# infergo-ml/gogp

Hardware: AMD Instinct MI355X
Metric: GP.Observe+Gradient evals/sec (fp64) at N=16384 D=8 (higher is better)
Workload: dtype f64

## Files before the change

gogp_amd/_lib.py:

```python
from __future__ import annotations

import ctypes
import os
import subprocess

from .kernel import CDesc

_HERE = os.path.dirname(os.path.abspath(__file__))
LIB_PATH = os.path.join(_HERE, "libgogp_hip.so")
HOOKS_PATH = os.path.join(_HERE, "libgogp_testhooks.so")

GOGP_OK, GOGP_EARG, GOGP_ENOTPD, GOGP_EHIP, GOGP_ESTATE, GOGP_ENOMEM, GOGP_ECOND = 0, 1, 2, 3, 4, 5, 6
GOGP_MAX_CANDIDATES = 16
GOGP_BATCH_MAX_N = 128
GOGP_COV_MAX_M = 4096
GOGP_MULTI_MAX_T = 128
GOGP_SPARSE_MAX_M = 4096

_dp = ctypes.POINTER(ctypes.c_double)
_i64 = ctypes.c_int64
_h = ctypes.c_void_p
_descp = ctypes.POINTER(CDesc)
GOGP_UNIQUE_ID_BYTES = 128


class CXfer(ctypes.Structure):
    _fields_ = [("peer", ctypes.c_int32), ("is_send", ctypes.c_int32), ("buf", ctypes.c_void_p),
                ("bytes", ctypes.c_int64)]


EXCHANGE_FN = ctypes.CFUNCTYPE(ctypes.c_int, ctypes.c_void_p, ctypes.POINTER(CXfer), ctypes.c_int32)
ALLREDUCE_FN = ctypes.CFUNCTYPE(ctypes.c_int, ctypes.c_void_p, ctypes.POINTER(ctypes.c_double),
                                ctypes.c_int64)
class CGemmOpts(ctypes.Structure):
    _fields_ = [(n, ctypes.c_int32) for n in ("ktri", "krag0", "new_row0", "kbeg0", "small_below", "prio", "rule",
                                              "tpb_shift", "rblk0", "cblk0", "pr", "Pr", "pc", "Pc", "beta0", "k")]
    _fields_ += [("bstride", ctypes.c_int64)]
    DEFAULTS = dict(ktri=0, krag0=-1, new_row0=-1, kbeg0=0, small_below=384, prio=0, rule=0, tpb_shift=0, rblk0=0,
                    cblk0=0, pr=0, Pr=1, pc=0, Pc=1, beta0=-1, k=1, bstride=0)


class CKParams(ctypes.Structure):
    _T, _D, _E = 4, 64, 32
    _fields_ = [("ndim", ctypes.c_int32), ("nterms", ctypes.c_int32), ("kind", ctypes.c_int32 * _T),
                ("ard", ctypes.c_int32 * _T), ("c", ctypes.c_double * _T), ("w", ctypes.c_double * _T),
                ("inv_len", (ctypes.c_double * _D) * _T), ("noise_var", ctypes.c_double), ("dnoise", ctypes.c_double),
                ("nevents", ctypes.c_int32), ("ev_axis", ctypes.c_int32), ("ev_from", ctypes.c_double * _E),
                ("ev_to", ctypes.c_double * _E), ("ev_disc", ctypes.c_double * _E)]


GOGP_TEST_NACC = 16 + 64


class CGemmPlan(ctypes.Structure):
    _fields_ = [("tile", ctypes.c_int32), ("waves", ctypes.c_int32), ("grid_x", ctypes.c_int64),
                ("grid_z", ctypes.c_int64), ("flops", ctypes.c_double), ("tag", ctypes.c_int64)]


SYMBOLS = [
    ("gogp_desc_check", ctypes.c_int, [_descp]),
    ("gogp_desc_ntheta_noise", ctypes.c_int, [_descp]),
    ("gogp_create", ctypes.c_int, [_descp, ctypes.c_int, ctypes.POINTER(_h)]),
    ("gogp_destroy", None, [_h]),
    ("gogp_last_error", ctypes.c_char_p, [_h]),
    ("gogp_notpd_index", _i64, [_h]),
    ("gogp_graph_info", ctypes.c_int, [_h, ctypes.POINTER(ctypes.c_int64), ctypes.POINTER(ctypes.c_int)]),
    ("gogp_events_check", ctypes.c_int, [_dp, ctypes.c_int, ctypes.c_int, ctypes.c_int]),
    ("gogp_set_events", ctypes.c_int, [_h, _dp, ctypes.c_int, ctypes.c_int]),
    ("gogp_set_data", ctypes.c_int, [_h, _dp, _dp, _i64]),
    ("gogp_set_data_device", ctypes.c_int, [_h, ctypes.c_void_p, ctypes.c_void_p, _i64]),
    ("gogp_absorb", ctypes.c_int, [_h, _dp, _dp]),
    ("gogp_observe", ctypes.c_int, [_h, _dp, _i64, _dp]),
# ... 200 lines not shown
```

gogp_amd/csrc/api.hip:

```cpp
#include <math.h>
#include <stdio.h>
#include <stdlib.h>
#include <string.h>

#include <algorithm>
#include <initializer_list>
#include <mutex>
#include <new>
#include <thread>
#include <type_traits>
#include <utility>

#include "handle.h"

using namespace gogp;

static thread_local std::string g_create_error;

extern "C" int gogp_desc_ntheta_noise(const gogp_desc *d) {
  return (d && (d->noise_kind == GOGP_NOISE_UNIFORM || d->noise_kind == GOGP_NOISE_CONSTANT_PARAM)) ? 1 : 0;
}

extern "C" int gogp_desc_check(const gogp_desc *d) {
  if (!d) return GOGP_EARG;
// ... 616 lines not shown
        ldc1[b] = PANEL;
        K1[b] = d * PANEL;
        A2[b] = Dinv + (size_t)i * PANEL * PANEL;
        lda2[b] = PANEL;
        B2[b] = C1[b];
        ldb2[b] = PANEL;
        C2[b] = X + (int64_t)i * PANEL * tld + (int64_t)j * PANEL;
        ldc2[b] = tld;
        K2[b] = PANEL;
      }
      launch_blockmm(sp, nb, A1, lda1, B1, ldb1, C1, ldc1, K1, 1.0);
      launch_blockmm(sp, nb, A2, lda2, B2, ldb2, C2, ldc2, K2, -1.0);
    }
  }
}

template <class T>
struct InvBufs {
  T *A, *Y;
  const T *L, *Dinv;
};
template <class T>
static void trtri_superstep(gogp_handle *h, const InvBufs<T> &B, const SuperPanel &P, hipStream_t st, hipStream_t s2) {
  const int64_t npad = h->npad, ld = npad;
  T *R = B.A, *Y = B.Y;
  const T *L = B.L;
  GemmProfile *pf = &h->prof;
  const int P0 = P.P0;
  const int64_t C0 = P.C0(), CE = P.CE();
  for (int q = 0; q < P.nsub; ++q) {
    const int p = P0 + q;
    const int64_t c0 = (int64_t)p * PANEL, c2 = c0 + PANEL;
    const T *Dp = B.Dinv + (size_t)p * PANEL * PANEL;
    launch_ydiag(st, Dp, Y + c0 * ld + c0, ld);
    if (c2 < CE)
      launch_zero_block(st, Y + c2 * ld + c0, ld, CE - c2, PANEL);
    if (c0 > 0) {
      GemmGrid gtri = chain_grid(h);
      gtri.ktri = h->ktri;
      launch_gemm_nt(st, GEMM_RECT, (int)(c0 / TILE), 2, PANEL, 1.0, R + c0, ld, Dp, PANEL, 0.0,
                      Y + c0, ld, pf, &gtri);
    }
    if (c2 < CE) {
      const InnerGroup g = inner_group(q, c2, CE);
      GemmGrid gch = chain_grid(h);
      if (h->krag) gch.krag0 = (int)(g.k0 / TILE);
      launch_gemm_nt(st, GEMM_RECT, (int)(c2 / TILE), (int)((g.ce - c2) / TILE), (int64_t)g.grp * PANEL,
                      -1.0, Y + g.k0, ld, L + c2 * ld + g.k0, ld, 1.0, R + c2, ld, pf, &gch);
    }
  }
  order(h, EV_BASE + 4 * P0 + 2, st, s2);
  const int nt = (int)((npad - CE) / TILE);
  if (nt > 0) {
    const int64_t Kw = CE - C0;
    const int mr = (int)(CE / TILE);
    const int ntn = nt < 2 * P.next_nsub ? nt : 2 * P.next_nsub;
    if (P0 > 0 && st != s2)
      (void)gogp::rec_stream_wait(st, ev(h, EV_BASE + 4 * P.prevP0 + 3));
    GemmGrid gch = chain_grid(h), gbulk;
    if (h->krag) gch.krag0 = gbulk.krag0 = (int)(C0 / TILE);
    launch_gemm_nt(st, GEMM_RECT, mr, ntn, Kw, -1.0, Y + C0, ld, L + CE * ld + C0, ld, 1.0,
                    R + CE, ld, pf, &gch);
    if (nt > ntn) {
      const int64_t C3 = CE + (int64_t)ntn * TILE;
      launch_gemm_nt(s2, GEMM_RECT, mr, nt - ntn, Kw, -1.0, Y + C0, ld, L + C3 * ld + C0, ld, 1.0,
                      R + C3, ld, pf, &gbulk);
    }
    (void)gogp::rec_event_record(ev(h, EV_BASE + 4 * P0 + 3), s2);
  }
}

static inline bool mixed_gradient(const gogp_handle *h) {
  return h->grad_prec == 32 && h->prec == 64 && !h->batch_mode && !h->dist;
}
static int ensure_g32(gogp_handle *h) {
  const int64_t cap = std::max(h->npad, h->cap_npad);
  if (h->g32A && h->g32_cap >= cap) return GOGP_OK;
  (void)hipFree(h->g32A);
  (void)hipFree(h->g32L);
  (void)hipFree(h->g32Y);
  (void)hipFree(h->g32D);
  h->g32A = h->g32L = h->g32Y = h->g32D = nullptr;
  h->g32_cap = 0;
  const size_t nn = (size_t)cap * (size_t)cap * sizeof(float);
  HIPCHK(h, hipMalloc(&h->g32A, nn));
  HIPCHK(h, hipMalloc(&h->g32L, nn));
  HIPCHK(h, hipMalloc(&h->g32Y, nn));
  HIPCHK(h, hipMalloc(&h->g32D, (size_t)(cap / PANEL) * PANEL * PANEL * sizeof(float)));
  h->g32_cap = cap;
  return GOGP_OK;
}
static void mixed_superstep(gogp_handle *h, const SuperPanel &P, hipStream_t st, hipStream_t s2) {
  const int64_t npad = h->npad, ld = npad, C0 = P.C0(), W = P.CE() - C0;
  launch_convert_block(st, h->bufL + C0 * ld + C0, ld, h->g32L + C0 * ld + C0, ld, (int)(npad - C0), (int)W);
  launch_convert_block(st, h->Dinv + (size_t)P.P0 * PANEL * PANEL, PANEL, h->g32D + (size_t)P.P0 * PANEL * PANEL, PANEL,
                       (int)W, PANEL);
  const InvBufs<float> B{h->g32A, h->g32Y, h->g32L, h->g32D};
  trtri_superstep<float>(h, B, P, st, s2);
}

template <class T>
static void kinv_accumulate(gogp_handle *h, const T *Y, T *A, int64_t C0, int64_t CE) {
  (void)gogp::rec_stream_wait(h->sk, ev(h, EV_BASE + 4 * (size_t)(C0 / PANEL) + 2));
  GemmGrid gk;
  gk.new_row0 = (int)(C0 / TILE);
  if (h->krag) gk.krag0 = (int)(C0 / TILE);
  launch_gemm_nt(h->sk, GEMM_LOWER, (int)(CE / TILE), (int)(CE / TILE), CE - C0, 1.0, Y + C0, h->npad, Y + C0, h->npad,
                 1.0, A, h->npad, &h->prof, &gk);
}

template <class T>
static void zero_inverse_rhs(gogp_handle *h, bool mixed, hipStream_t s) {
  if (mixed)
    launch_zero_upper_blocks(s, h->g32A, h->npad, h->npad);
  else
    launch_zero_upper_blocks(s, reinterpret_cast<T *>(h->bufA), h->npad, h->npad);
}
template <class T>
static void inverse_superstep(gogp_handle *h, bool mixed, const SuperPanel &P, hipStream_t st, hipStream_t s2,
                              bool fuse_kinv) {
  if (mixed) {
    mixed_superstep(h, P, st, s2);
    if (fuse_kinv) kinv_accumulate<float>(h, h->g32Y, h->g32A, P.C0(), P.CE());
  } else {
    const InvBufs<T> B{reinterpret_cast<T *>(h->bufA), reinterpret_cast<T *>(h->bufY), reinterpret_cast<const T *>(h->bufL),
                       reinterpret_cast<const T *>(h->Dinv)};
    trtri_superstep<T>(h, B, P, st, s2);
    if (fuse_kinv) kinv_accumulate<T>(h, B.Y, B.A, P.C0(), P.CE());
  }
}

static inline int chain_split_of(const gogp_handle *h, bool eager) {
  if (h->dist || h->prec != 64) return 0;
  if (h->chain_split >= 0) return h->chain_split;
  return (h->npad <= 8192 || !eager) ? 2 : 0;
}
static void fused_panel(gogp_handle *h, hipStream_t sp, double *A, double *L, int64_t ld, int64_t c0, int64_t npad,
                        GemmProfile *pf) {
  const int64_t c1 = c0 + TILE, c2 = c0 + PANEL;
  const int mt1 = (int)((npad - c1) / TILE);
  const GemmGrid gch = chain_grid(h);
  launch_panel128_slabs(sp, A + c0 * ld + c0, ld, L + c0 * ld + c0, ld, 0, npad - c1, c0, h->n, h->info, h->chain_slabs);
  launch_gemm_nt(sp, GEMM_RECT, mt1, 1, TILE, -1.0, L + c1 * ld + c0, ld, L + c1 * ld + c0, ld, 1.0, A + c1 * ld + c1, ld,
                 pf, &gch);
  launch_panel128_slabs(sp, A + c0 * ld + c0, ld, L + c0 * ld + c0, ld, 1, npad - c2, c0, h->n, h->info, h->chain_slabs);
}

static void begin_evaluation(gogp_handle *h, std::initializer_list<hipStream_t> streams) {
  auto wait = [&](int e) {
    for (hipStream_t q : streams) (void)gogp::rec_stream_wait(q, ev(h, e));
  };
// ... 43 lines not shown
  bool fuse_kinv = eager && (h->kinv_fused < 0 ? (npad <= 10240 || mixed) : h->kinv_fused != 0);
  int split = fp32 ? 0 : chain_split_of(h, eager);

  void d64_init(hipStream_t q, int first, int nblk) const {
    if constexpr (fp32)
      launch_widen_diag_blocks(q, A + (int64_t)first * PANEL * (ld + 1), ld, h->D64 + (size_t)first * PANEL * PANEL, nblk);
  }
  void d64_update(hipStream_t q, int64_t k0, int64_t K, int first, int nblk) const {
    if constexpr (fp32) {
      if (h->d64_active)
        launch_diag_syrk_f64(q, L + (int64_t)first * PANEL * ld + k0, ld, K, h->D64 + (size_t)first * PANEL * PANEL, nblk);
    }
  }

  int build_gram() const {
    if (sp != s) order(h, EV_ENTRY, s, sp);
    HIPCHK(h, cand_memset(h, h->info, sizeof(long long), sp));
    const int w0 = superpanel_width(h, npanel, 0);
    {
      AuxTimer tm(h, GOGP_PROF_GRAM, s);
      launch_gram_lower_split(sp, s, h->devP, h->D, h->dX, h->n, npad, A, ld, (int64_t)w0 * PANEL, h->ev());
    }
    h->d64_active = fp32 && h->diag_fp64 != 0;
    if (h->d64_active) {
      const int rc = ensure_d64(h);
      if (rc != GOGP_OK) return rc;
      d64_init(sp, 0, w0);
      if (npanel > w0) d64_init(s, w0, npanel - w0);
    }
    (void)gogp::rec_event_record(ev(h, EV_GRAM), s);
    if (eager) {
      (void)gogp::rec_stream_wait(s2, ev(h, EV_GRAM));
      (void)gogp::rec_stream_wait(st, ev(h, EV_GRAM));
      zero_inverse_rhs<T>(h, mixed, s2);
      order(h, EV_INIT, s2, st);
    }
    return GOGP_OK;
  }

  void chain_superpanel(const SuperPanel &P) const {
    const int64_t CE = P.CE();
    for (int q = 0; q < P.nsub; ++q) {
      const int p = P.P0 + q;
      const int64_t c0 = (int64_t)p * PANEL, c2 = c0 + PANEL;
      if constexpr (!fp32) {
        if (split) fused_panel(h, sp, A, L, ld, c0, npad, pf);
      }
      if (!split) {
        T *Dp = Dinv + (size_t)p * PANEL * PANEL;
        diag_block(h, sp, A + c0 * ld + c0, ld, L + c0 * ld + c0, ld, Dp, c0);
        const int mt2 = (int)((npad - c2) / TILE);
        if (mt2 > 0) {
          GemmGrid gtri = chain_grid(h);
          gtri.ktri = h->ktri;
          launch_gemm_nt(sp, GEMM_RECT, mt2, 2, PANEL, 1.0, A + c2 * ld + c0, ld, Dp, PANEL, 0.0,
                          L + c2 * ld + c0, ld, pf, &gtri);
        }
      }
      if (c2 < CE) {
        d64_update(sp, c0, PANEL, p + 1, (int)((CE - c2) / PANEL));
        const InnerGroup g = inner_group(q, c2, CE);
        const GemmGrid gch = chain_grid(h);
        launch_gemm_nt(sp, GEMM_TRAP, (int)((npad - c2) / TILE), (int)((g.ce - c2) / TILE),
                        (int64_t)g.grp * PANEL, -1.0, L + c2 * ld + g.k0, ld, L + c2 * ld + g.k0, ld, 1.0,
                        A + c2 * ld + c2, ld, pf, &gch);
      }
    }
  }
// ... 230 lines not shown
  h->with_obs = true;
  return observe_theta(h, x, lml);
}

extern "C" int gogp_lml(gogp_handle *h, double *lml) {
  if (!h || !lml) return GOGP_EARG;
  if (h->n == 0) {
    *lml = 0.0;
    return GOGP_OK;
  }
  if (!h->factored) return fail(h, GOGP_ESTATE, "LML: nothing absorbed");
  *lml = h->lml;
  return GOGP_OK;
}

template <class T>
static int compute_kinv_t(gogp_handle *h) {
  if (h->have_kinv) return GOGP_OK;
  const int64_t npad = h->npad, ld = npad;
  hipStream_t s = h->s;
  GemmProfile *pf = &h->prof;
  if (h->kinv_pending) {
    (void)gogp::rec_stream_wait(s, ev(h, EV_KINV));
    if (h->trtri_pending) (void)gogp::rec_stream_wait(s, ev(h, EV_TRTRI));
    h->kinv_pending = h->trtri_pending = false;
    h->have_kinv = true;
    return GOGP_OK;
  }
  const bool mixed = std::is_same<T, double>::value && mixed_gradient(h);
  if (!h->trtri_done) {
    hipStream_t sp = h->lookahead ? h->sp : h->s;
    const int rcy = mixed ? ensure_g32(h) : ensure_y(h);
    if (rcy != GOGP_OK) return rcy;
    zero_inverse_rhs<T>(h, mixed, s);
    order(h, EV_INIT, s, sp);
    for (const SuperPanel &P : superpanels(h)) inverse_superstep<T>(h, mixed, P, sp, s, false);
    order(h, EV_TRTRI, sp, s);
    h->trtri_done = true;
  } else if (h->trtri_pending) {
    (void)gogp::rec_stream_wait(s, ev(h, h->ydone_valid ? EV_YDONE : EV_TRTRI));
  }
  if (mixed) {
    launch_gemm_nt(s, GEMM_LAUUM, h->nblk, h->nblk, npad, 1.0, h->g32Y, ld, h->g32Y, ld, 0.0, h->g32A, ld, pf);
  } else {
    GemmGrid gk;
    if (h->kinv_c1 > 0) {
      (void)gogp::rec_stream_wait(s, ev(h, EV_KINV));
      gk.kbeg0 = (int)h->kinv_c1;
    }
    launch_gemm_nt(s, GEMM_LAUUM, h->nblk, h->nblk, npad, 1.0, reinterpret_cast<const T *>(h->bufY), ld,
                   reinterpret_cast<const T *>(h->bufY), ld, 0.0, reinterpret_cast<T *>(h->bufA), ld, pf, &gk);
  }
  if (h->trtri_pending && h->ydone_valid) (void)gogp::rec_stream_wait(s, ev(h, EV_TRTRI));
  h->trtri_pending = false;
  h->have_kinv = true;
  return GOGP_OK;
}
static int compute_kinv(gogp_handle *h) {
  return h->prec == 32 ? compute_kinv_t<float>(h) : compute_kinv_t<double>(h);
}

static int64_t grad_len(const gogp_handle *h) {
  return h->with_obs ? h->P + h->n * (h->D + 1) : h->P;
}

static void assemble_gradient(const gogp_handle *h, const double *a, double dnoise, double *out) {
  const gogp_desc &d = h->desc;
// ... 2369 lines not shown
```

gogp_amd/csrc/common.h:

```cpp
#pragma once
#include <hip/hip_runtime.h>
#include <stdint.h>

#include <string>
#include <vector>

#include "../../include/gogp_hip.h"
#include "graphrec.h"

namespace gogp {

constexpr int TILE = 128;
constexpr int PANEL = 256;
constexpr int GEMM_BK = 16;

struct DevParams {
  int ndim, nterms, ns, nn;
  int kind[GOGP_MAX_TERMS];
  int ard[GOGP_MAX_TERMS];
  double c[GOGP_MAX_TERMS];
  double w[GOGP_MAX_TERMS];
  double inv_len[GOGP_MAX_TERMS][GOGP_MAX_NDIM];
  double noise_var;
  double dnoise;
  int nevents, ev_axis;
  double ev_from[GOGP_MAX_EVENTS], ev_to[GOGP_MAX_EVENTS], ev_disc[GOGP_MAX_EVENTS];
};

constexpr int ACC_TRACE = 3 * GOGP_MAX_TERMS;
constexpr int ACC_ARD0 = 16;
constexpr int NACC = ACC_ARD0 + GOGP_MAX_NDIM;

struct Batch {
  int k = 1;
  long stride = 0;
};
inline thread_local Batch tl_batch;
template <class P>
__device__ __forceinline__ P *cand(P *p, long bstride) {
  return (P *)((const char *)p + (long)blockIdx.z * bstride);
}

struct GemmProfile {
  bool on = false;
  std::vector<hipEvent_t> pool;
  size_t used = 0;
  double flops = 0;
  int64_t launches = 0;
  std::vector<double> lflops;
  std::vector<int64_t> ltag;
};

struct GemmGrid {
  int rule = 0, tpb_shift = 0, rblk0 = 0, cblk0 = 0, pr = 0, Pr = 1, pc = 0, Pc = 1, beta0 = -1;
  int new_row0 = -1;
  int ktri = 0;
  int prio = 0;
  int krag0 = -1;
  int small_below = 384;
  int kbeg0 = 0;
};

struct BlockMap {
  int nb_shift = 9, pr = 0, Pr = 1, pc = 0, Pc = 1;
  __host__ __device__ long grow(long lrow) const {
    const long nbm = (1L << nb_shift) - 1;
    return ((((lrow >> nb_shift) * Pr + pr)) << nb_shift) + (lrow & nbm);
  }
  __host__ __device__ long gcol(long lcol) const {
    const long nbm = (1L << nb_shift) - 1;
    return ((((lcol >> nb_shift) * Pc + pc)) << nb_shift) + (lcol & nbm);
  }
};

#ifdef GOGP_WGSTAMP
struct StampRec {
  long long base, nwg, tag, stream;
};
constexpr int STAMP_SLOTS = 8;
extern unsigned long long *g_stamp_buf;
extern long long g_stamp_cap, g_stamp_used, g_stamp_nrec;
extern StampRec g_stamp_rec[1 << 16];
unsigned long long *stamp_reserve(long long nwg, long long tag, hipStream_t s);
#endif

enum GemmMode { GEMM_RECT = 0, GEMM_LOWER = 1, GEMM_LAUUM = 2,
                GEMM_TRAP = 3 };

void launch_dgemm_nt(hipStream_t s, GemmMode mode, int mt, int nt, int64_t K,
                     double alpha, const double *A, int64_t lda, const double *B,
                     int64_t ldb, double beta, double *C, int64_t ldc,
                     GemmProfile *prof, const GemmGrid *grid = nullptr);

void launch_gemm_nt(hipStream_t s, GemmMode mode, int mt, int nt, int64_t K, double alpha, const double *A,
                    int64_t lda, const double *B, int64_t ldb, double beta, double *C, int64_t ldc,
                    GemmProfile *prof, const GemmGrid *grid = nullptr);
void launch_gemm_nt(hipStream_t s, GemmMode mode, int mt, int nt, int64_t K, double alpha, const float *A,
                    int64_t lda, const float *B, int64_t ldb, double beta, float *C, int64_t ldc,
                    GemmProfile *prof, const GemmGrid *grid = nullptr);
void launch_gram_lower_split(hipStream_t s_first, hipStream_t s_rest, const DevParams *p, int ndim,
                             const double *X, int64_t n, int64_t npad, float *K, int64_t ld,
                             int64_t wcols, bool ev = false);
void launch_cross(hipStream_t s, const DevParams *p, int ndim, const double *X, int64_t n,
                  int64_t npad, const double *Z, int64_t m, int64_t mpad, float *KsT, int64_t ld, bool ev = false);
void launch_trsv_fwd_step(hipStream_t s, const float *L, int64_t ld, const float *Dinv, int b, int nblk,
                          double *y, double *z);
void launch_trsv_bwd_step(hipStream_t s, const float *L, int64_t ld, const float *Dinv, int b, int nblk,
                          double *zwork, double *alpha);
void launch_lml_scalars(hipStream_t s, const float *L, int64_t ld, const double *z, const double *y,
                        const double *alpha, int64_t n, double *scalars);
void launch_alpha_from_y(hipStream_t s, const float *Y, int64_t ld, const double *z, int64_t npad,
                         double *alpha);
void launch_rownorm_dot(hipStream_t s, const float *V, int64_t ld, const double *vec, int64_t ncols,
                        int64_t m, double *dot, double *sq);
void launch_zero_upper_blocks(hipStream_t s, float *R, int64_t ld, int64_t npad);
void launch_zero_block(hipStream_t s, float *B, int64_t ld, int64_t rows, int64_t cols);
void launch_ydiag(hipStream_t s, const float *Dinv, float *Ydiag, int64_t ld);
void launch_extract_lower(hipStream_t s, const float *L, int64_t ld, int64_t n, double *out);
void launch_pack_lower(hipStream_t s, const double *in, int64_t n, int64_t npad, float *L, int64_t ld);
void launch_convert_block(hipStream_t s, const float *src, int64_t lds_, double *dst, int64_t ldd, int rows,
                          int cols);
void launch_convert_block(hipStream_t s, const double *src, int64_t lds_, float *dst, int64_t ldd, int rows,
                          int cols);
void launch_grad_reduce(hipStream_t s, const DevParams *p, int ndim, int ard_dims, const double *X,
                        const double *alpha, const float *Kinv, int64_t ld, int64_t n, int64_t npad,
                        double *partials, double *out, bool radial1 = false, int mfma_min_dims = 1, bool ev = false,
                        int max_blocks = 0);

void launch_gram_lower(hipStream_t s, const DevParams *p, int ndim, const double *X,
                       int64_t n, int64_t npad, double *K, int64_t ld, bool ev = false);
void launch_gram_local(hipStream_t s, const DevParams *p, int ndim, const double *X, int64_t n,
                       int64_t mrows, int64_t ncols, BlockMap map, double *K, int64_t ld, bool ev = false);
void launch_gram_local(hipStream_t s, const DevParams *p, int ndim, const double *X, int64_t n,
                       int64_t mrows, int64_t ncols, BlockMap map, float *K, int64_t ld, bool ev = false);
void launch_gram_lower_split(hipStream_t s_first, hipStream_t s_rest, const DevParams *p, int ndim,
                             const double *X, int64_t n, int64_t npad, double *K, int64_t ld,
                             int64_t wcols, bool ev = false);
void launch_cross(hipStream_t s, const DevParams *p, int ndim, const double *X, int64_t n,
                  int64_t npad, const double *Z, int64_t m, int64_t mpad, double *KsT,
                  int64_t ld, bool ev = false);
void launch_residual(hipStream_t s, const DevParams *p, int ndim, const double *X, int64_t n, int64_t npad,
                     const double *v, const double *y, double *part, int nslab, double *r, bool radial1 = false,
                     bool ev = false);
void launch_kmatvec_share(hipStream_t s, const DevParams *p, int ndim, const double *X, int64_t n, int64_t npad,
                          const double *v, int part_idx, int nparts, double *part, int nslab, double *out,
                          bool radial1 = false, bool ev = false);
void launch_prior(hipStream_t s, const DevParams *p, const double *Z, int64_t m,
                  double *prior);

void launch_trsv_fwd_step(hipStream_t s, const double *L, int64_t ld, const double *Dinv,
// ... 49 lines not shown
void launch_pcov_add_mu(hipStream_t s, const double *G, int64_t ldg, const double *mu, int64_t ns, int64_t m, double *out);
int grad_reduce_blocks(int64_t npad);

void launch_grad_reduce(hipStream_t s, const DevParams *p, int ndim, int ard_dims,
                        const double *X, const double *alpha, const double *Kinv, int64_t ld, int64_t n,
                        int64_t npad, double *partials, double *out, bool radial1 = false, int mfma_min_dims = 1,
                        bool ev = false, int max_blocks = 0);
int grad_reduce_blocks_local(int64_t mrows, int64_t ncols);
void launch_grad_reduce_local(hipStream_t s, const DevParams *p, int ndim, int ard_dims,
                              const double *X, const double *alpha, const double *Kinv, int64_t ld,
                              int64_t n, int64_t mrows, int64_t ncols, BlockMap map, double *partials,
                              double *out, bool radial1 = false, int mfma_min_dims = 1, bool ev = false,
                              int max_blocks = 0);
void launch_grad_reduce_local(hipStream_t s, const DevParams *p, int ndim, int ard_dims,
                              const double *X, const double *alpha, const float *Kinv, int64_t ld,
                              int64_t n, int64_t mrows, int64_t ncols, BlockMap map, double *partials,
                              double *out, bool radial1 = false, int mfma_min_dims = 1, bool ev = false,
                              int max_blocks = 0);

void launch_grad_ard_mfma(hipStream_t s, const DevParams *p, int ndim, const double *X, const double *alpha,
                          const double *Kinv, int64_t ld, int64_t n, int nt, int ntc, int ntiles, int blocks,
                          BlockMap map, double *partials);
void launch_grad_ard_mfma(hipStream_t s, const DevParams *p, int ndim, const double *X, const double *alpha,
                          const float *Kinv, int64_t ld, int64_t n, int nt, int ntc, int ntiles, int blocks,
                          BlockMap map, double *partials);

void launch_xgrad(hipStream_t s, const DevParams *p, int ndim, const double *X,
                  const double *alpha, double *Kinv, int64_t ld, int64_t n, int64_t npad,
                  double *gx, bool ev = false);

void launch_rownorm_dot(hipStream_t s, const double *V, int64_t ld, const double *vec,
                        int64_t ncols, int64_t m, double *dot, double *sq);

void launch_zero_upper_blocks(hipStream_t s, double *R, int64_t ld, int64_t npad);
void launch_alpha_from_y(hipStream_t s, const double *Y, int64_t ld, const double *z,
                         int64_t npad, double *alpha);
void launch_zero_block(hipStream_t s, double *B, int64_t ld, int64_t rows, int64_t cols);
void launch_ydiag(hipStream_t s, const double *Dinv, double *Ydiag, int64_t ld);
void launch_tinv_init(hipStream_t s, const double *Dinv, double *X, double *XT, int nsub, int64_t tld);
void launch_tinv_init(hipStream_t s, const float *Dinv, float *X, float *XT, int nsub, int64_t tld);
void launch_blockmm(hipStream_t s, int nprod, const double *const *A, const int64_t *lda, const double *const *B,
                    const int64_t *ldb, double *const *C, const int64_t *ldc, const int *K, double alpha);
void launch_blockmm(hipStream_t s, int nprod, const float *const *A, const int64_t *lda, const float *const *B,
                    const int64_t *ldb, float *const *C, const int64_t *ldc, const int *K, double alpha);
void launch_trace_from_y(hipStream_t s, const float *Y, int64_t ld, int64_t n, int64_t npad, const double *alpha,
                         double *part, double *out);
size_t trsm_small_workspace_bytes(int64_t npad);
void launch_trsm_small(hipStream_t s, const double *L, int64_t ld, const double *Dinv, const double *KsT, int64_t ldk,
                       int64_t npad, int j0, int cnt, void *ws, double *dq, unsigned **tmo_dev);
void launch_trsm_small(hipStream_t s, const float *L, int64_t ld, const float *Dinv, const float *KsT, int64_t ldk,
                       int64_t npad, int j0, int cnt, void *ws, double *dq, unsigned **tmo_dev);
enum { TS_SOL_PAIRED = 0, TS_SOL_COMPACT = 1, TS_SOL_GRANULE = 2, TS_SOL_ROWS = 3 };
struct TsSolution {
  const void *p = nullptr;
  int kind = TS_SOL_PAIRED, width = 32;
};
TsSolution trsm_small_solution(int64_t npad, int j0, int cnt, void *ws, bool f32 = false);
constexpr int APPEND_PART = 64 * 64 + 64;
void launch_append_gram(hipStream_t s, TsSolution v0, TsSolution v1, int m0, int m, int64_t npc, int64_t n,
                        const double *z, double *part, double *Lnew, int64_t ld);
void launch_append_commit(hipStream_t s, const DevParams *p, const double *X2, const double *y2, int m, int64_t n,
                          const double *part, int nslab, double *Lnew, int64_t ld, double *z2out, long long *info,
                          bool ev);
void launch_append_identity_rows(hipStream_t s, double *L, int64_t ld, int64_t r0, int64_t r1, int64_t ncols);
void launch_append_restride(hipStream_t s, const double *src, int64_t ld0, int64_t npad0, double *dst, int64_t ld1,
                            int64_t npad1);
constexpr int REMOVE_W = 32, REMOVE_W_SMALL = 4;
void launch_remove_gather(hipStream_t s, const double *src, int64_t ld0, const int *map, int64_t n1, double *dst,
                          int64_t npad1);
void launch_remove_rows(hipStream_t s, const double *src, const int *map, int64_t n1, int width, double *dst);
void launch_remove_w(hipStream_t s, const double *src, int64_t ld0, const int *map, const int *rem, int mc, int mw, int64_t r0,
// ... 63 lines not shown
```

gogp_amd/csrc/gemm_plan.h:

```cpp
#pragma once
#include <algorithm>

#include "common.h"

namespace gogp {

struct GemmPrecision {
  int kstep;
  bool band_513_768;
  bool cand_batch;
  bool lauum_kbeg0;
};
constexpr int SGEMM_BK = 32;
constexpr GemmPrecision GEMM_F64 = {GEMM_BK, true, true, true}, GEMM_F32 = {SGEMM_BK, false, false, false};

struct GemmPlan {
  int mt, nt, nkt, kend, trap, rule, tpb_shift, rblk0, cblk0, pr, Pr, pc, Pc, beta0, new_row0, ktri, prio, krag0;
  int kbeg0;
  GemmMode mode;
  int ntiles;
  double flops;
  int64_t tag;
  int tile, waves;
  unsigned gridx, gridz;
};

inline GemmPlan gemm_plan(GemmMode mode, int mt, int nt, int64_t K, const GemmGrid *grid, int ncand, GemmPrecision prec) {
  constexpr int NONE = 0x7fffffff;
  GemmPlan p{};
  if (!prec.cand_batch) ncand = 1;
  p.mt = mt;
  p.nt = nt;
  p.nkt = (int)(K / prec.kstep);
  p.kend = (int)K;
  p.trap = mode == GEMM_TRAP;
  p.rule = p.tpb_shift = p.rblk0 = p.cblk0 = p.pr = p.pc = p.beta0 = 0;
  p.Pr = p.Pc = 1;
  p.new_row0 = (mode == GEMM_LOWER && grid && grid->new_row0 >= 0) ? grid->new_row0 : NONE;
  p.ktri = (mode == GEMM_RECT && grid && grid->ktri) ? 1 : 0;
  p.prio = grid ? grid->prio : 0;
  p.krag0 = (mode != GEMM_LAUUM && mode != GEMM_TRAP && grid && grid->krag0 >= 0 && !p.ktri) ? grid->krag0 : NONE;
  p.kbeg0 = (mode == GEMM_LAUUM && grid && prec.lauum_kbeg0) ? grid->kbeg0 : 0;
  if (grid && grid->rule) {
    p.rule = grid->rule;
    p.tpb_shift = grid->tpb_shift;
    p.rblk0 = grid->rblk0;
    p.cblk0 = grid->cblk0;
    p.pr = grid->pr;
    p.Pr = grid->Pr;
    p.pc = grid->pc;
    p.Pc = grid->Pc;
    p.beta0 = grid->beta0;
  }
  int ntiles;
  double flops;
  if (mode == GEMM_TRAP) {
    mode = GEMM_RECT;
    ntiles = mt * nt;
    const int nb = nt / 2;
    flops = 2.0 * TILE * TILE * (double)K * ((double)mt * nt - 4.0 * nb * (nb - 1) / 2.0);
  } else if (mode == GEMM_RECT) {
    ntiles = mt * nt;
    flops = 2.0 * (double)mt * TILE * (double)nt * TILE * (double)K;
    if (p.ktri) {
      flops = 0;
      for (int j = 0; j < nt; ++j)
        flops += 2.0 * (double)mt * TILE * TILE * (double)std::min<int64_t>(K, (int64_t)(j + 1) * TILE);
    }
    if (p.krag0 != NONE) {
      flops = 0;
      for (int i = 0; i < mt; ++i)
// ... 51 lines not shown
```

gogp_amd/csrc/gemm_tile.h:

```cpp
#pragma once
#include <type_traits>

#include <hip/hip_ext.h>

#include "common.h"
#include "gemm_plan.h"

namespace gogp {

template <class T>
struct GemmArgsCommon {
  const T *A;
  const T *B;
  T *C;
  long lda, ldb, ldc;
  int mt, nt;
  int nkt;
  T alpha, beta;
  int kend;
  int trap;
  int rule, tpb_shift, rblk0, cblk0, pr, Pr, pc, Pc, beta0;
  int new_row0;
  int ktri;
  int prio;
// ... 22 lines not shown
#endif
}
__device__ __forceinline__ void wait_vmcnt0() {
#if defined(__HIP_DEVICE_COMPILE__)
  __builtin_amdgcn_s_waitcnt(0x0F70);
#endif
}

__device__ __forceinline__ int xcd_chunk(int t) {
  const int nwg = gridDim.x;
  const int q = nwg >> 3, r = nwg & 7;
  const int xcd = t & 7;
  return (xcd < r ? xcd * (q + 1) : r * (q + 1) + (xcd - r) * q) + (t >> 3);
}

template <int BT, int BK, class T>
__device__ __forceinline__ bool rect_tile_assignment(const GemmArgs<T> &g, int &ti_out, int &tj_out, T &beta_out,
                                                     int &kbeg_out, int &nkt_out) {
  int t = blockIdx.x;
  if (!g.rule) t = xcd_chunk(t);
  int ti, tj;
  if (g.rule) {
    const int x = t & 7, slot = t >> 3;
    const int rr = slot / g.nt;
    ti = x + 8 * rr;
    tj = slot - rr * g.nt;
    if (ti >= g.mt) return false;
  } else {
    ti = t / g.nt;
    tj = t - ti * g.nt;
    if (g.trap && (tj * BT) / PANEL > (ti * BT) / PANEL) return false;
  }
  T beta = g.beta;
  if (g.rule) {
    const int gI = (g.rblk0 + (ti >> g.tpb_shift)) * g.Pr + g.pr;
    const int gJ = (g.cblk0 + (tj >> g.tpb_shift)) * g.Pc + g.pc;
    const int msk = (1 << g.tpb_shift) - 1;
    if (gI < gJ || (gI == gJ && (ti & msk) < (tj & msk))) return false;
    if (g.rule == 2) beta = (gI == g.beta0) ? T(0) : T(1);
  }
  int kbeg = 0, nkt = g.nkt;
  if (g.ktri) nkt = min(nkt, (tj + 1) * BT / BK);
  if (ti > g.krag0) {
    kbeg = (ti - g.krag0) * BT;
    nkt -= kbeg / BK;
  }
  ti_out = ti, tj_out = tj, beta_out = beta, kbeg_out = kbeg, nkt_out = nkt;
  return true;
}

template <class T>
struct TileKernel;

template <class T>
void launch_tile_gemm(hipStream_t s, GemmMode mode, int mt, int nt, int64_t K, double alpha, const T *A, int64_t lda,
                      const T *B, int64_t ldb, double beta, T *C, int64_t ldc, GemmProfile *prof, const GemmGrid *grid) {
  if (mt <= 0 || nt <= 0 || K <= 0) return;
  constexpr bool F64 = std::is_same_v<T, double>;
  const GemmPlan p = gemm_plan(mode, mt, nt, K, grid, tl_batch.k, F64 ? GEMM_F64 : GEMM_F32);
  GemmArgs<T> g;
  g.A = A;
  g.B = B;
  g.C = C;
  g.lda = lda;
  g.ldb = ldb;
  g.ldc = ldc;
// ... 47 lines not shown
```

gogp_amd/csrc/solve.hip:

```cpp
#include "common.h"

namespace gogp {

__device__ __forceinline__ void load8(const double *p, double *o) {
  const double2 *q = reinterpret_cast<const double2 *>(p);
  const double2 a = q[0], b = q[1], c = q[2], d = q[3];
  o[0] = a.x; o[1] = a.y; o[2] = b.x; o[3] = b.y; o[4] = c.x; o[5] = c.y; o[6] = d.x; o[7] = d.y;
}
__device__ __forceinline__ void load8(const float *p, double *o) {
  const float4 *q = reinterpret_cast<const float4 *>(p);
  const float4 a = q[0], b = q[1];
  o[0] = a.x; o[1] = a.y; o[2] = a.z; o[3] = a.w; o[4] = b.x; o[5] = b.y; o[6] = b.z; o[7] = b.w;
}
__device__ __forceinline__ void load2(const double *p, double &a, double &b) {
  const double2 v = *reinterpret_cast<const double2 *>(p);
  a = v.x;
  b = v.y;
}
__device__ __forceinline__ void load2(const float *p, double &a, double &b) {
  const float2 v = *reinterpret_cast<const float2 *>(p);
  a = v.x;
  b = v.y;
}
__device__ __forceinline__ void store2zero(double *p) {
// ... 288 lines not shown
  const long q0 = (i / PANEL) * PANEL;
  const T *row = Y + i * ld;
  double b = 0.0;
  for (long q = q0 + threadIdx.x; q < ncols; q += 256) {
    const double v = (double)row[q];
    b += v * v;
  }
  b = wave_sum(b);
  if ((threadIdx.x & 63) == 0) red[threadIdx.x >> 6] = b;
  __syncthreads();
  if (threadIdx.x == 0) part[i] = alpha[i] * alpha[i] - ((red[0] + red[1]) + (red[2] + red[3]));
}
__global__ __launch_bounds__(1024) void sum_kernel(const double *__restrict__ v, long n, double *__restrict__ out) {
  __shared__ double red[16];
  double a = 0.0;
  for (long i = threadIdx.x; i < n; i += 1024) a += v[i];
  a = wave_sum(a);
  if ((threadIdx.x & 63) == 0) red[threadIdx.x >> 6] = a;
  __syncthreads();
  if (threadIdx.x == 0) {
    double t = 0.0;
    for (int w = 0; w < 16; ++w) t += red[w];
    out[0] = t;
  }
}
void launch_trace_from_y(hipStream_t s, const float *Y, int64_t ld, int64_t n, int64_t npad, const double *alpha,
                         double *part, double *out) {
  if (n <= 0) return;
  GOGP_KLAUNCH(trace_rows_kernel<float>, dim3((unsigned)n), dim3(256), 0, s, Y, (long)ld, (long)npad, alpha, part);
  GOGP_KLAUNCH(sum_kernel, dim3(1), dim3(1024), 0, s, (const double *)part, (long)n, out);
}

template <class T>
__global__ __launch_bounds__(256) void zero_upper_kernel(T *__restrict__ R, long ld,
                                                         long npad, long bstride) {
  R = cand(R, bstride);
  const long row = blockIdx.y;
  const long cstart = (row / PANEL + 1) * PANEL;
  const long c = cstart + ((long)blockIdx.x * 256 + threadIdx.x) * 2;
  if (c >= npad) return;
  store2zero(R + row * ld + c);
}

void launch_zero_upper_blocks(hipStream_t s, double *R, int64_t ld, int64_t npad) {
  if (npad <= PANEL) return;
  dim3 grid((unsigned)((npad / 2 + 255) / 256), (unsigned)(npad - PANEL), (unsigned)tl_batch.k);
  GOGP_KLAUNCH(zero_upper_kernel<double>, grid, dim3(256), 0, s, R, (long)ld, (long)npad,
                     tl_batch.stride);
}
void launch_zero_upper_blocks(hipStream_t s, float *R, int64_t ld, int64_t npad) {
  if (npad <= PANEL) return;
  dim3 grid((unsigned)((npad / 2 + 255) / 256), (unsigned)(npad - PANEL));
  GOGP_KLAUNCH(zero_upper_kernel<float>, grid, dim3(256), 0, s, R, (long)ld, (long)npad, 0L);
}

template <class T>
__global__ __launch_bounds__(256) void ydiag_kernel(const T *__restrict__ Dinv,
                                                    T *__restrict__ Y, long ld, long bstride) {
  Dinv = cand(Dinv, bstride);
  Y = cand(Y, bstride);
  __shared__ T tile[32][33];
  const int bx = blockIdx.x & 7, by = blockIdx.x >> 3;
  const int tx = threadIdx.x & 31, ty = threadIdx.x >> 5;
#pragma unroll
  for (int r = 0; r < 32; r += 8) tile[ty + r][tx] = Dinv[(by * 32 + ty + r) * 256 + bx * 32 + tx];
  __syncthreads();
#pragma unroll
  for (int r = 0; r < 32; r += 8) Y[(long)(bx * 32 + ty + r) * ld + by * 32 + tx] = tile[tx][ty + r];
}

void launch_ydiag(hipStream_t s, const double *Dinv, double *Ydiag, int64_t ld) {
  GOGP_KLAUNCH(ydiag_kernel<double>, dim3(64, 1, (unsigned)tl_batch.k), dim3(256), 0, s, Dinv, Ydiag,
                     (long)ld, tl_batch.stride);
}
void launch_ydiag(hipStream_t s, const float *Dinv, float *Ydiag, int64_t ld) {
  GOGP_KLAUNCH(ydiag_kernel<float>, dim3(64), dim3(256), 0, s, Dinv, Ydiag, (long)ld, 0L);
}

template <class T>
__global__ __launch_bounds__(256) void tinv_init_kernel(const T *__restrict__ Dinv, T *__restrict__ X,
                                                        T *__restrict__ XT, int nsub, long tld, long bstride) {
  Dinv = cand(Dinv, bstride);
  X = cand(X, bstride);
  if (XT) XT = cand(XT, bstride);
  __shared__ T tile[32][33];
  const int tpr = nsub * 8;
  const int bx = blockIdx.x % tpr, by = blockIdx.x / tpr;
  const int I = by >> 3, J = bx >> 3;
  const int tx = threadIdx.x & 31, ty = threadIdx.x >> 5;
  const long r0 = (long)by * 32, c0 = (long)bx * 32;
  if (I == J) {
    const T *D = Dinv + (long)I * 256 * 256 + (long)(by & 7) * 32 * 256 + (bx & 7) * 32;
#pragma unroll
    for (int r = 0; r < 32; r += 8) {
      const T v = D[(ty + r) * 256 + tx];
      X[(r0 + ty + r) * tld + c0 + tx] = v;
      tile[ty + r][tx] = v;
    }
    if (XT) {
      __syncthreads();
      const long tr0 = (long)I * 256 + (long)(bx & 7) * 32, tc0 = (long)I * 256 + (long)(by & 7) * 32;
#pragma unroll
      for (int r = 0; r < 32; r += 8) XT[(tr0 + ty + r) * tld + tc0 + tx] = tile[tx][ty + r];
    }
  } else if (I < J) {
#pragma unroll
    for (int r = 0; r < 32; r += 8) X[(r0 + ty + r) * tld + c0 + tx] = (T)0;
  } else if (XT) {
#pragma unroll
// ... 486 lines not shown
```

gogp_amd/csrc/testhooks.hip:

```cpp
#include <cstdlib>
#include <cstring>
#include <stdio.h>

#include "common.h"
#include "gemm_plan.h"
#include "../../include/gogp_testhooks.h"

struct gogp_handle;
namespace gogp {
int dist_init_replay(gogp_handle *h, int rank, int nranks, int prow, int pcol);
}
extern "C" int gogp_test_dist_init_replay(void *h, int rank, int nranks, int prow, int pcol) {
  return gogp::dist_init_replay(static_cast<gogp_handle *>(h), rank, nranks, prow, pcol);
}

namespace gogp_th {
void launch_diag256(hipStream_t s, const double *A, int64_t ld, double *Lout, int64_t ldl,
                    double *Dinv, int64_t row0, int64_t nvalid, long long *info);
void launch_diag256_stamped(hipStream_t s, const double *A, double *Lout, double *Dinv,
                            long long *info, unsigned long long *stamps);
void launch_panel128_stamped(hipStream_t s, const double *A, double *Lout, int64_t rows_below, long long *info,
                             unsigned long long *stamps);
}

// ... 175 lines not shown
  if (e == hipSuccess) {
    launch_dgemm_nt(0, GEMM_RECT, (int)(M / TILE), (int)(N / TILE), K, alpha, dA, K, dB, K, beta,
                    dC, N, nullptr);
    e = hipDeviceSynchronize();
  }
  if (e == hipSuccess) e = hipMemcpy(C, dC, (size_t)M * N * sizeof(double), hipMemcpyDeviceToHost);
  (void)hipFree(dA);
  (void)hipFree(dB);
  (void)hipFree(dC);
  return e == hipSuccess ? GOGP_OK : GOGP_EHIP;
}

namespace {
bool covers(int64_t len, int64_t off, int64_t ld, int64_t rows, int64_t cols, int64_t k, int64_t stride) {
  if (len <= 0 || off < 0 || ld < cols || rows <= 0 || cols <= 0 || k <= 0 || stride < 0) return false;
  const int64_t hi = off + (k - 1) * stride + (rows - 1) * ld + cols;
  return hi <= len;
}
bool device_ok(int device) {
  int ndev = 0;
  if (hipGetDeviceCount(&ndev) != hipSuccess || ndev <= 0) return false;
  return device < 0 || hipSetDevice(device) == hipSuccess;
}
bool gemm_launch_args_ok(int precision, int mode, int mt, int nt, int64_t K, const gogp_test_gemm_opts &o) {
  if (precision != 64 && precision != 32) return false;
  if (mode < GEMM_RECT || mode > GEMM_TRAP || mt <= 0 || nt <= 0 || K <= 0) return false;
  const int64_t kstep = precision == 64 ? GEMM_BK : SGEMM_BK, al = 16 / (precision / 8);
  if (K % kstep || K > (1 << 30)) return false;
  if ((mode == GEMM_LOWER || mode == GEMM_LAUUM) && mt != nt) return false;
  if (o.k < 1 || o.k > 64 || o.bstride < 0 || o.bstride % al || (o.k > 1 && o.bstride == 0)) return false;
  if (precision == 32 && (o.k > 1 || o.kbeg0 != 0)) return false;
  if (o.kbeg0 < 0 || o.kbeg0 % kstep || o.kbeg0 > K || (o.kbeg0 && mode != GEMM_LAUUM)) return false;
  if (o.new_row0 < -1 || (o.new_row0 >= 0 && mode != GEMM_LOWER)) return false;
  if (o.ktri && mode != GEMM_RECT) return false;
  if (o.krag0 < -1 || (o.krag0 >= 0 && (o.ktri || (mode != GEMM_RECT && mode != GEMM_LOWER)))) return false;
  if (o.krag0 >= 0 && o.krag0 < mt && K < (int64_t)(mt - o.krag0) * TILE) return false;
  if (o.rule < 0 || o.rule > 2 || (o.rule && mode != GEMM_RECT)) return false;
  if (o.rule && (o.tpb_shift < 0 || o.tpb_shift > 8 || o.rblk0 < 0 || o.cblk0 < 0 || o.Pr < 1 || o.Pc < 1 ||
                 o.pr < 0 || o.pr >= o.Pr || o.pc < 0 || o.pc >= o.Pc))
    return false;
  return true;
}
const gogp_test_gemm_opts GEMM_OPTS_DEFAULT = {0, -1, -1, 0, 384, 0, 0, 0, 0, 0, 0, 1, 0, 1, -1, 1, 0};
GemmGrid gemm_grid_of(const gogp_test_gemm_opts &o) {
  GemmGrid g;
  g.ktri = o.ktri;
  g.krag0 = o.krag0;
  g.new_row0 = o.new_row0;
  g.kbeg0 = o.kbeg0;
  g.small_below = o.small_below;
  g.prio = o.prio;
  g.rule = o.rule;
  g.tpb_shift = o.tpb_shift;
  g.rblk0 = o.rblk0;
  g.cblk0 = o.cblk0;
  g.pr = o.pr;
  g.Pr = o.Pr;
  g.pc = o.pc;
  g.Pc = o.Pc;
  g.beta0 = o.beta0;
  return g;
}
}

extern "C" int gogp_test_gemm_plan(int precision, int mode, int mt, int nt, int64_t K, const gogp_test_gemm_opts *opt,
                                   gogp_test_gemm_plan_out *out) {
  const gogp_test_gemm_opts o = opt ? *opt : GEMM_OPTS_DEFAULT;
  if (!out || !gemm_launch_args_ok(precision, mode, mt, nt, K, o)) return GOGP_EARG;
  const GemmGrid g = gemm_grid_of(o);
  const GemmPlan p = gemm_plan((GemmMode)mode, mt, nt, K, &g, o.k, precision == 64 ? GEMM_F64 : GEMM_F32);
  out->tile = p.tile;
  out->waves = p.waves;
  out->grid_x = p.gridx;
  out->grid_z = p.gridz;
  out->flops = p.flops;
  out->tag = p.tag;
  return GOGP_OK;
}

extern "C" int gogp_test_gemm_nt(int device, int precision, int mode, int mt, int nt, int64_t K, double alpha,
                                 double beta, const void *A, int64_t a_len, int64_t a_off, int64_t lda, const void *B,
// ... 1175 lines not shown
```

include/gogp_testhooks.h:

```cpp
#ifndef GOGP_TESTHOOKS_H
#define GOGP_TESTHOOKS_H

#include <stdint.h>

#include "gogp_hip.h"

#ifdef __cplusplus
extern "C" {
#endif

int gogp_mfma_f64_peak(int device, int iters, double *tflops, double *cyc_per_mfma,
                       double *clock_mhz);
int gogp_mfma_f32_peak(int device, int iters, double *tflops, double *cyc_per_mfma,
                       double *clock_mhz);

int gogp_test_dgemm_nt(int device, int64_t M, int64_t N, int64_t K, double alpha,
                       const double *A, const double *B, double beta, double *C);

typedef struct gogp_test_gemm_opts {
  int32_t ktri, krag0, new_row0, kbeg0, small_below, prio;
  int32_t rule, tpb_shift, rblk0, cblk0, pr, Pr, pc, Pc, beta0;
  int32_t k;
  int64_t bstride;
} gogp_test_gemm_opts;

int gogp_test_gemm_nt(int device, int precision, int mode, int mt, int nt, int64_t K, double alpha, double beta,
                      const void *A, int64_t a_len, int64_t a_off, int64_t lda, const void *B, int64_t b_len,
                      int64_t b_off, int64_t ldb, void *C, int64_t c_len, int64_t c_off, int64_t ldc,
                      const gogp_test_gemm_opts *opt);

typedef struct gogp_test_gemm_plan_out {
  int32_t tile, waves;
  int64_t grid_x, grid_z;
  double flops;
  int64_t tag;
} gogp_test_gemm_plan_out;
int gogp_test_gemm_plan(int precision, int mode, int mt, int nt, int64_t K, const gogp_test_gemm_opts *opt,
                        gogp_test_gemm_plan_out *out);

int gogp_test_diag_syrk(int device, int bs, const float *L, int64_t l_len, int64_t l_off, int64_t ld, int64_t K,
                        int64_t row_stride, double *D64, int64_t d_len, int nblocks);

int gogp_test_diag256_product(int device, int variant, const double *A, int64_t ld, double *L, int64_t ldl,
                              double *Dinv, int64_t row0, int64_t nvalid, long long *info);


int64_t gogp_test_trsm_small_workspace(int64_t npad);

int gogp_test_trsm_small(int device, int precision, int64_t npad, const void *L, int64_t l_len, int64_t ld,
                         const void *Dinv, const void *KsT, int64_t k_len, int64_t ldk, int j0, int cnt, double *dq,
                         int64_t dq_len, void *sol, int64_t sol_len, int *kind, int *width, int64_t *sol_off,
                         unsigned *tmo);

int gogp_test_trsv_steps(int device, int precision, int dir, int64_t npad, const void *L, int64_t l_len, int64_t ld,
                         const void *Dinv, int b0, int b1, int k, int64_t bstride, double *w, int64_t w_len, double *out,
                         int64_t out_len);
// ... 113 lines not shown
```

Measured before the change: 14.02.

## Replace upper-block zeroing with beta=0 on new rows in RECT GEMMs

Removes the full-matrix zero_upper_blocks pass that cleared the strictly-upper panel blocks of the inverse workspace before the triangular inverse. RECT GEMMs now take a rect_new_row0 threshold so tiles at or below that row use beta=0 and overwrite instead of accumulating into uninitialised memory. The per-panel zero_block launch is folded into the ydiag kernel as extra workgroups, except when krag is on. This removes one large memory-write pass and some launches, but correctness now depends on every previously zeroed region being written with beta=0 before it is read.

```diff
diff --git a/gogp_amd/_lib.py b/gogp_amd/_lib.py
--- a/gogp_amd/_lib.py
+++ b/gogp_amd/_lib.py
@@ -35,9 +35,9 @@
 class CGemmOpts(ctypes.Structure):
     _fields_ = [(n, ctypes.c_int32) for n in ("ktri", "krag0", "new_row0", "kbeg0", "small_below", "prio", "rule",
                                               "tpb_shift", "rblk0", "cblk0", "pr", "Pr", "pc", "Pc", "beta0", "k")]
-    _fields_ += [("bstride", ctypes.c_int64)]
+    _fields_ += [("bstride", ctypes.c_int64), ("rect_new_row0", ctypes.c_int32)]
     DEFAULTS = dict(ktri=0, krag0=-1, new_row0=-1, kbeg0=0, small_below=384, prio=0, rule=0, tpb_shift=0, rblk0=0,
-                    cblk0=0, pr=0, Pr=1, pc=0, Pc=1, beta0=-1, k=1, bstride=0)
+                    cblk0=0, pr=0, Pr=1, pc=0, Pc=1, beta0=-1, k=1, bstride=0, rect_new_row0=-1)
 
 
 class CKParams(ctypes.Structure):
diff --git a/gogp_amd/csrc/api.hip b/gogp_amd/csrc/api.hip
--- a/gogp_amd/csrc/api.hip
+++ b/gogp_amd/csrc/api.hip
@@ -672,9 +672,7 @@
     const int p = P0 + q;
     const int64_t c0 = (int64_t)p * PANEL, c2 = c0 + PANEL;
     const T *Dp = B.Dinv + (size_t)p * PANEL * PANEL;
-    launch_ydiag(st, Dp, Y + c0 * ld + c0, ld);
-    if (c2 < CE)
-      launch_zero_block(st, Y + c2 * ld + c0, ld, CE - c2, PANEL);
+    launch_ydiag(st, Dp, Y + c0 * ld + c0, ld, h->krag ? 0 : CE - c2);
     if (c0 > 0) {
       GemmGrid gtri = chain_grid(h);
       gtri.ktri = h->ktri;
@@ -685,6 +683,7 @@
       const InnerGroup g = inner_group(q, c2, CE);
       GemmGrid gch = chain_grid(h);
       if (h->krag) gch.krag0 = (int)(g.k0 / TILE);
+      gch.rect_new_row0 = (int)(g.k0 / TILE);
       launch_gemm_nt(st, GEMM_RECT, (int)(c2 / TILE), (int)((g.ce - c2) / TILE), (int64_t)g.grp * PANEL,
                       -1.0, Y + g.k0, ld, L + c2 * ld + g.k0, ld, 1.0, R + c2, ld, pf, &gch);
     }
@@ -699,6 +698,7 @@
       (void)gogp::rec_stream_wait(st, ev(h, EV_BASE + 4 * P.prevP0 + 3));
     GemmGrid gch = chain_grid(h), gbulk;
     if (h->krag) gch.krag0 = gbulk.krag0 = (int)(C0 / TILE);
+    gch.rect_new_row0 = gbulk.rect_new_row0 = (int)(C0 / TILE);
     launch_gemm_nt(st, GEMM_RECT, mr, ntn, Kw, -1.0, Y + C0, ld, L + CE * ld + C0, ld, 1.0,
                     R + CE, ld, pf, &gch);
     if (nt > ntn) {
@@ -750,13 +750,6 @@
 }
 
 template <class T>
-static void zero_inverse_rhs(gogp_handle *h, bool mixed, hipStream_t s) {
-  if (mixed)
-    launch_zero_upper_blocks(s, h->g32A, h->npad, h->npad);
-  else
-    launch_zero_upper_blocks(s, reinterpret_cast<T *>(h->bufA), h->npad, h->npad);
-}
-template <class T>
 static void inverse_superstep(gogp_handle *h, bool mixed, const SuperPanel &P, hipStream_t st, hipStream_t s2,
                               bool fuse_kinv) {
   if (mixed) {
@@ -866,8 +859,6 @@
     if (eager) {
       (void)gogp::rec_stream_wait(s2, ev(h, EV_GRAM));
       (void)gogp::rec_stream_wait(st, ev(h, EV_GRAM));
-      zero_inverse_rhs<T>(h, mixed, s2);
-      order(h, EV_INIT, s2, st);
     }
     return GOGP_OK;
   }
@@ -1164,7 +1155,6 @@
     hipStream_t sp = h->lookahead ? h->sp : h->s;
     const int rcy = mixed ? ensure_g32(h) : ensure_y(h);
     if (rcy != GOGP_OK) return rcy;
-    zero_inverse_rhs<T>(h, mixed, s);
     order(h, EV_INIT, s, sp);
     for (const SuperPanel &P : superpanels(h)) inverse_superstep<T>(h, mixed, P, sp, s, false);
     order(h, EV_TRTRI, sp, s);
diff --git a/gogp_amd/csrc/common.h b/gogp_amd/csrc/common.h
--- a/gogp_amd/csrc/common.h
+++ b/gogp_amd/csrc/common.h
@@ -54,6 +54,7 @@
 struct GemmGrid {
   int rule = 0, tpb_shift = 0, rblk0 = 0, cblk0 = 0, pr = 0, Pr = 1, pc = 0, Pc = 1, beta0 = -1;
   int new_row0 = -1;
+  int rect_new_row0 = -1;
   int ktri = 0;
   int prio = 0;
   int krag0 = -1;
@@ -113,9 +114,8 @@
                          double *alpha);
 void launch_rownorm_dot(hipStream_t s, const float *V, int64_t ld, const double *vec, int64_t ncols,
                         int64_t m, double *dot, double *sq);
-void launch_zero_upper_blocks(hipStream_t s, float *R, int64_t ld, int64_t npad);
 void launch_zero_block(hipStream_t s, float *B, int64_t ld, int64_t rows, int64_t cols);
-void launch_ydiag(hipStream_t s, const float *Dinv, float *Ydiag, int64_t ld);
+void launch_ydiag(hipStream_t s, const float *Dinv, float *Ydiag, int64_t ld, int64_t zero_rows_below = 0);
 void launch_extract_lower(hipStream_t s, const float *L, int64_t ld, int64_t n, double *out);
 void launch_pack_lower(hipStream_t s, const double *in, int64_t n, int64_t npad, float *L, int64_t ld);
 void launch_convert_block(hipStream_t s, const float *src, int64_t lds_, double *dst, int64_t ldd, int rows,
@@ -231,11 +231,10 @@
 void launch_rownorm_dot(hipStream_t s, const double *V, int64_t ld, const double *vec,
                         int64_t ncols, int64_t m, double *dot, double *sq);
 
-void launch_zero_upper_blocks(hipStream_t s, double *R, int64_t ld, int64_t npad);
 void launch_alpha_from_y(hipStream_t s, const double *Y, int64_t ld, const double *z,
                          int64_t npad, double *alpha);
 void launch_zero_block(hipStream_t s, double *B, int64_t ld, int64_t rows, int64_t cols);
-void launch_ydiag(hipStream_t s, const double *Dinv, double *Ydiag, int64_t ld);
+void launch_ydiag(hipStream_t s, const double *Dinv, double *Ydiag, int64_t ld, int64_t zero_rows_below = 0);
 void launch_tinv_init(hipStream_t s, const double *Dinv, double *X, double *XT, int nsub, int64_t tld);
 void launch_tinv_init(hipStream_t s, const float *Dinv, float *X, float *XT, int nsub, int64_t tld);
 void launch_blockmm(hipStream_t s, int nprod, const double *const *A, const int64_t *lda, const double *const *B,
diff --git a/gogp_amd/csrc/gemm_plan.h b/gogp_amd/csrc/gemm_plan.h
--- a/gogp_amd/csrc/gemm_plan.h
+++ b/gogp_amd/csrc/gemm_plan.h
@@ -36,7 +36,9 @@
   p.trap = mode == GEMM_TRAP;
   p.rule = p.tpb_shift = p.rblk0 = p.cblk0 = p.pr = p.pc = p.beta0 = 0;
   p.Pr = p.Pc = 1;
-  p.new_row0 = (mode == GEMM_LOWER && grid && grid->new_row0 >= 0) ? grid->new_row0 : NONE;
+  p.new_row0 = (mode == GEMM_LOWER && grid && grid->new_row0 >= 0)        ? grid->new_row0
+               : (mode == GEMM_RECT && grid && grid->rect_new_row0 >= 0) ? grid->rect_new_row0
+                                                                         : NONE;
   p.ktri = (mode == GEMM_RECT && grid && grid->ktri) ? 1 : 0;
   p.prio = grid ? grid->prio : 0;
   p.krag0 = (mode != GEMM_LAUUM && mode != GEMM_TRAP && grid && grid->krag0 >= 0 && !p.ktri) ? grid->krag0 : NONE;
diff --git a/gogp_amd/csrc/gemm_tile.h b/gogp_amd/csrc/gemm_tile.h
--- a/gogp_amd/csrc/gemm_tile.h
+++ b/gogp_amd/csrc/gemm_tile.h
@@ -78,6 +78,7 @@
     if (g.trap && (tj * BT) / PANEL > (ti * BT) / PANEL) return false;
   }
   T beta = g.beta;
+  if (ti >= g.new_row0) beta = T(0);
   if (g.rule) {
     const int gI = (g.rblk0 + (ti >> g.tpb_shift)) * g.Pr + g.pr;
     const int gJ = (g.cblk0 + (tj >> g.tpb_shift)) * g.Pc + g.pc;
diff --git a/gogp_amd/csrc/solve.hip b/gogp_amd/csrc/solve.hip
--- a/gogp_amd/csrc/solve.hip
+++ b/gogp_amd/csrc/solve.hip
@@ -344,29 +344,6 @@
 }
 
 template <class T>
-__global__ __launch_bounds__(256) void zero_upper_kernel(T *__restrict__ R, long ld,
-                                                         long npad, long bstride) {
-  R = cand(R, bstride);
-  const long row = blockIdx.y;
-  const long cstart = (row / PANEL + 1) * PANEL;
-  const long c = cstart + ((long)blockIdx.x * 256 + threadIdx.x) * 2;
-  if (c >= npad) return;
-  store2zero(R + row * ld + c);
-}
-
-void launch_zero_upper_blocks(hipStream_t s, double *R, int64_t ld, int64_t npad) {
-  if (npad <= PANEL) return;
-  dim3 grid((unsigned)((npad / 2 + 255) / 256), (unsigned)(npad - PANEL), (unsigned)tl_batch.k);
-  GOGP_KLAUNCH(zero_upper_kernel<double>, grid, dim3(256), 0, s, R, (long)ld, (long)npad,
-                     tl_batch.stride);
-}
-void launch_zero_upper_blocks(hipStream_t s, float *R, int64_t ld, int64_t npad) {
-  if (npad <= PANEL) return;
-  dim3 grid((unsigned)((npad / 2 + 255) / 256), (unsigned)(npad - PANEL));
-  GOGP_KLAUNCH(zero_upper_kernel<float>, grid, dim3(256), 0, s, R, (long)ld, (long)npad, 0L);
-}
-
-template <class T>
 __global__ __launch_bounds__(256) void ydiag_kernel(const T *__restrict__ Dinv,
                                                     T *__restrict__ Y, long ld, long bstride) {
   Dinv = cand(Dinv, bstride);
@@ -374,6 +351,11 @@
   __shared__ T tile[32][33];
   const int bx = blockIdx.x & 7, by = blockIdx.x >> 3;
   const int tx = threadIdx.x & 31, ty = threadIdx.x >> 5;
+  if (by >= 8) {
+#pragma unroll
+    for (int r = 0; r < 32; r += 8) Y[(long)(by * 32 + ty + r) * ld + bx * 32 + tx] = T(0);
+    return;
+  }
 #pragma unroll
   for (int r = 0; r < 32; r += 8) tile[ty + r][tx] = Dinv[(by * 32 + ty + r) * 256 + bx * 32 + tx];
   __syncthreads();
@@ -381,12 +363,14 @@
   for (int r = 0; r < 32; r += 8) Y[(long)(bx * 32 + ty + r) * ld + by * 32 + tx] = tile[tx][ty + r];
 }
 
-void launch_ydiag(hipStream_t s, const double *Dinv, double *Ydiag, int64_t ld) {
-  GOGP_KLAUNCH(ydiag_kernel<double>, dim3(64, 1, (unsigned)tl_batch.k), dim3(256), 0, s, Dinv, Ydiag,
+void launch_ydiag(hipStream_t s, const double *Dinv, double *Ydiag, int64_t ld, int64_t zero_rows_below) {
+  const unsigned nwg = 64 + 8 * (unsigned)(zero_rows_below / 32);
+  GOGP_KLAUNCH(ydiag_kernel<double>, dim3(nwg, 1, (unsigned)tl_batch.k), dim3(256), 0, s, Dinv, Ydiag,
                      (long)ld, tl_batch.stride);
 }
-void launch_ydiag(hipStream_t s, const float *Dinv, float *Ydiag, int64_t ld) {
-  GOGP_KLAUNCH(ydiag_kernel<float>, dim3(64), dim3(256), 0, s, Dinv, Ydiag, (long)ld, 0L);
+void launch_ydiag(hipStream_t s, const float *Dinv, float *Ydiag, int64_t ld, int64_t zero_rows_below) {
+  const unsigned nwg = 64 + 8 * (unsigned)(zero_rows_below / 32);
+  GOGP_KLAUNCH(ydiag_kernel<float>, dim3(nwg), dim3(256), 0, s, Dinv, Ydiag, (long)ld, 0L);
 }
 
 template <class T>
diff --git a/gogp_amd/csrc/testhooks.hip b/gogp_amd/csrc/testhooks.hip
--- a/gogp_amd/csrc/testhooks.hip
+++ b/gogp_amd/csrc/testhooks.hip
@@ -231,6 +231,7 @@
   if (precision == 32 && (o.k > 1 || o.kbeg0 != 0)) return false;
   if (o.kbeg0 < 0 || o.kbeg0 % kstep || o.kbeg0 > K || (o.kbeg0 && mode != GEMM_LAUUM)) return false;
   if (o.new_row0 < -1 || (o.new_row0 >= 0 && mode != GEMM_LOWER)) return false;
+  if (o.rect_new_row0 < -1 || (o.rect_new_row0 >= 0 && mode != GEMM_RECT)) return false;
   if (o.ktri && mode != GEMM_RECT) return false;
   if (o.krag0 < -1 || (o.krag0 >= 0 && (o.ktri || (mode != GEMM_RECT && mode != GEMM_LOWER)))) return false;
   if (o.krag0 >= 0 && o.krag0 < mt && K < (int64_t)(mt - o.krag0) * TILE) return false;
@@ -240,12 +241,13 @@
     return false;
   return true;
 }
-const gogp_test_gemm_opts GEMM_OPTS_DEFAULT = {0, -1, -1, 0, 384, 0, 0, 0, 0, 0, 0, 1, 0, 1, -1, 1, 0};
+const gogp_test_gemm_opts GEMM_OPTS_DEFAULT = {0, -1, -1, 0, 384, 0, 0, 0, 0, 0, 0, 1, 0, 1, -1, 1, 0, -1};
 GemmGrid gemm_grid_of(const gogp_test_gemm_opts &o) {
   GemmGrid g;
   g.ktri = o.ktri;
   g.krag0 = o.krag0;
   g.new_row0 = o.new_row0;
+  g.rect_new_row0 = o.rect_new_row0;
   g.kbeg0 = o.kbeg0;
   g.small_below = o.small_below;
   g.prio = o.prio;
diff --git a/include/gogp_testhooks.h b/include/gogp_testhooks.h
--- a/include/gogp_testhooks.h
+++ b/include/gogp_testhooks.h
@@ -22,6 +22,7 @@
   int32_t rule, tpb_shift, rblk0, cblk0, pr, Pr, pc, Pc, beta0;
   int32_t k;
   int64_t bstride;
+  int32_t rect_new_row0;
 } gogp_test_gemm_opts;
 
 int gogp_test_gemm_nt(int device, int precision, int mode, int mt, int nt, int64_t K, double alpha, double beta,
```

After: 14.02, median of 2. About the same (+0.0%).
